# unlikeghost/DeepLearning-MPI

Hardware: AMD Instinct MI355X
Metric: images/sec (whole node) ResNet-50 DDP bs=256/GPU (higher is better)
Workload: dtype bf16; 1 GPU; model=resnet50, global_batch=256, image=224, in_channels=3, per_gpu_batch=256, parallelism=dp1, backend=single, device=cuda, optimizer=SGD(momentum=0.9, wd=1e-5), hipgraph=False

## Files before the change

deeplearning_mpi_amd/csrc/binding/conv_bwd.cpp:

```cpp
#include <c10/hip/HIPCachingAllocator.h>

#include <algorithm>
#include <vector>

#include "common.h"
#include "ops.h"

namespace dlmpi_ext {

using dlmpi::ConvArgs;
using dlmpi::ConvPhase;
using dlmpi::DgradStreamArgs;
using dlmpi::make_fastdiv;
using dlmpi::WgradArgs;

c10::optional<at::Tensor> conv2d_dgrad_pro(const at::Tensor& dy, int N, int P, int Q, int K, int lddy, int dyoff,
                                       const at::Tensor& wT, int C, int R, int S, int stride, int pad, int H, int W,
                                       at::Tensor dx, int lddx, int dxoff, const c10::optional<at::Tensor>& res,
                                       int ldres, int resoff, const c10::optional<at::Tensor>& mask, int ldmask,
                                       int maskoff, const c10::optional<at::Tensor>& z, int ldz, int zoff,
                                       const c10::optional<at::Tensor>& z2, int ldz2, int z2off,
                                       const c10::optional<at::Tensor>& mscale,
                                       const c10::optional<at::Tensor>& mshift,
                                       const c10::optional<at::Tensor>& mbits, bool colsum, int pro,
                                       const c10::optional<at::Tensor>& pk0, const c10::optional<at::Tensor>& pk1,
                                       const c10::optional<at::Tensor>& pz, int ldpz, int pzoff,
                                       const c10::optional<at::Tensor>& bias) {
  require_gpu(dy, "dy");
  if (stride > 2) throw std::runtime_error("conv2d_dgrad: stride <= 2 supported");
  if (bias.has_value() && bias->defined() && (bias->scalar_type() != at::kFloat || bias->numel() < C))
    throw std::runtime_error("conv2d_dgrad: bias must be fp32 [C]");
  ConvArgs a{};
  a.f32 = act_f32(dy, "conv2d_dgrad");
  same_type(dy, wT, "conv2d_dgrad wT");
  same_type(dy, dx, "conv2d_dgrad dx");
  same_type(dy, res, "conv2d_dgrad res");
  same_type(dy, mask, "conv2d_dgrad mask");
  same_type(dy, z, "conv2d_dgrad z");
  same_type(dy, z2, "conv2d_dgrad z2");
  a.x = ptr<uint16_t>(dy);
  a.H = P; a.W = Q; a.C = K; a.ldx = lddy; a.xoff = dyoff;
  a.w = ptr<uint16_t>(wT);
  a.ldw = R * S * K;
  a.S = S;
  a.OH = H; a.OW = W;
  a.so = stride; a.sa = 1;
  a.Nimg = N; a.Kout = C;
  fill_epilogue(a, dx, lddx, dxoff, bias, res, ldres, resoff, c10::nullopt, c10::nullopt, false, c10::nullopt);
  a.vec_store = ((lddx % 8) == 0 && (dxoff % 8) == 0) ? 1 : 0;
  a.mask = optr<uint16_t>(mask);
  a.ldmask = ldmask; a.maskoff = maskoff;
  a.z = optr<uint16_t>(z);
  a.ldz = ldz; a.zoff = zoff;
  a.z2 = optr<uint16_t>(z2);
  a.ldz2 = ldz2; a.z2off = z2off;
  a.mscale = optr<float>(mscale);
  a.mshift = optr<float>(mshift);
  a.mbits = optr<uint8_t>(mbits);
  if (a.mbits && (mbits->numel() != (int64_t)N * H * W * (C / 8) || C % 8))
    throw std::runtime_error("conv2d_dgrad: mask bits must be [N*H*W][C/8]");
  a.nstat = a.z2 ? 3 : 2;
  if (a.z && !a.mask && !a.mscale && !a.mbits)
    throw std::runtime_error("conv2d_dgrad: fused BN statistics need the ReLU mask");
  if (a.mscale && (!a.z || !a.mshift)) throw std::runtime_error("conv2d_dgrad: mask from z needs z, scale, shift");
// ... 32 lines not shown
        (a.z != nullptr) == (mode != 0) && a.vec_store && a.kvalid == C && (lddy | dyoff) % 8 == 0 &&
        (!a.res || (ldres | resoff) % 8 == 0) && fits(M, lddy) && fits(M, lddx) && (!a.res || fits(M, ldres)) &&
        (!a.z || fits(M, ldz)) && (!a.z2 || fits(M, ldz2)) && dx.scalar_type() == at::kBFloat16 &&
        dlmpi_dgrad_stream_plan(M, K, C, mode, a.z2 ? 1 : 0, a.res ? 1 : 0, &sbm, &sbn, &G)) {
      DgradStreamArgs sa{};
      sa.x = ptr<uint16_t>(dy);
      sa.ldx = lddy; sa.xoff = dyoff;
      sa.w = ptr<uint16_t>(wT);
      sa.y = reinterpret_cast<uint16_t*>(a.y);
      sa.ldy = lddx; sa.yoff = dxoff;
      sa.y_bytes = (int)std::min<int64_t>(INT32_MAX, (int64_t)dx.numel() * 2);
      sa.M = (int)M; sa.K = K; sa.Kout = C;
      sa.bias = a.bias;
      sa.res = static_cast<const uint16_t*>(a.res);
      sa.ldres = ldres; sa.resoff = resoff;
      sa.z = static_cast<const uint16_t*>(a.z);
      sa.ldz = ldz; sa.zoff = zoff;
      sa.z2 = static_cast<const uint16_t*>(a.z2);
      sa.ldz2 = ldz2; sa.z2off = z2off;
      sa.mbits = a.mbits;
      sa.mscale = a.mscale; sa.mshift = a.mshift;
      sa.G = G; sa.ntiles = C / sbn; sa.mtiles = (int)ceil_div(M, sbm);
      c10::optional<at::Tensor> st;
      if (a.z) {
        st = at::empty({(int64_t)G, (int64_t)a.nstat, (int64_t)C}, dy.options().dtype(at::kFloat));
        sa.stats = ptr<float>(*st);
      }
      check(dlmpi_conv1x1_dgrad_stream(&sa, sbm, sbn, mode, cur_stream()), "conv2d_dgrad (stream 1x1)");
      g_ran.dgrad_stream = 1;
      return st;
    }
  }
  set_kstep(a, K);
  set_prologue(a, pro, pk0, pk1, pz, ldpz, pzoff);
  TileQuery q{(int64_t)N * H * W / (stride * stride), C, (int64_t)R * S * K / (stride * stride), K, R, S, stride, pad,
              H, W, a.f32, pro};
  q.halo_ok = P == H && Q == W;
  q.pipe_ok = g_sw.pipe_dgrad != 0;
  const Tiles t = select_tiles(q);
  int bm = t.bm, bn = t.bn;
  const int pipe = t.pipe;
  const bool halo = t.halo;
  a.ntiles = ceil_div(C, bn);
  a.nphase = stride * stride;
  int tiles = 0;
  for (int ph = 0; ph < stride; ++ph) {
    for (int pw = 0; pw < stride; ++pw) {
      ConvPhase& p = a.ph[ph * stride + pw];
      const int r0 = (ph + pad) % stride, s0 = (pw + pad) % stride;
      p.P = (H - ph + stride - 1) / stride;
      p.Q = (W - pw + stride - 1) / stride;
      p.Tr = r0 < R ? (R - r0 + stride - 1) / stride : 0;
      p.Ts = s0 < S ? (S - s0 + stride - 1) / stride : 0;
// ... 29 lines not shown
  check(dlmpi_conv_igemm_ex(&a, bm, bn, pipe, cur_stream()), "conv2d_dgrad");
  return stats;
}

c10::optional<at::Tensor> conv2d_dgrad(const at::Tensor& dy, int N, int P, int Q, int K, int lddy, int dyoff,
                                       const at::Tensor& wT, int C, int R, int S, int stride, int pad, int H, int W,
                                       at::Tensor dx, int lddx, int dxoff, const c10::optional<at::Tensor>& res,
                                       int ldres, int resoff, const c10::optional<at::Tensor>& mask, int ldmask,
                                       int maskoff, const c10::optional<at::Tensor>& z, int ldz, int zoff,
                                       const c10::optional<at::Tensor>& z2, int ldz2, int z2off,
                                       const c10::optional<at::Tensor>& mscale,
                                       const c10::optional<at::Tensor>& mshift,
                                       const c10::optional<at::Tensor>& mbits, bool colsum) {
  return conv2d_dgrad_pro(dy, N, P, Q, K, lddy, dyoff, wT, C, R, S, stride, pad, H, W, dx, lddx, dxoff, res, ldres,
                          resoff, mask, ldmask, maskoff, z, ldz, zoff, z2, ldz2, z2off, mscale, mshift, mbits, colsum,
                          0, c10::nullopt, c10::nullopt, c10::nullopt, 0, 0, c10::nullopt);
}

struct PendingReduce {
  at::Tensor ws;
  hipStream_t s;
  dlmpi::WgradReduceEntry e;
};
static std::vector<PendingReduce> g_pending;
static bool g_wgrad_defer = false;
static int g_wgrad_batch = dlmpi::kWgradBatch;
static bool g_defer_direct = true;
static bool g_wgrad_bypass = false;
static int64_t g_reduce_launches = 0;

void wgrad_flush() {
// ... 200 lines not shown
```

deeplearning_mpi_amd/csrc/binding/conv_fwd.cpp:

```cpp
#include <algorithm>
#include <cstdio>
#include <map>
#include <vector>

#include "common.h"

namespace dlmpi_ext {

using dlmpi::ConvArgs;
using dlmpi::ConvPhase;
using dlmpi::FinArgs;
using dlmpi::Stream1x1Args;
using dlmpi::make_fastdiv;

void apply_halo(ConvArgs& a, int N, int bm) {
  ConvPhase& p = a.ph[0];
  int th = 8, tw = 16, tiles_h = 1, tiles_w = 1;
  halo_geom(p.P, p.Q, bm, th, tw, tiles_h, tiles_w);
  a.halo = 1;
  a.th = th;
  a.tw = tw;
  a.tiles_h = tiles_h;
  a.tiles_w = tiles_w;
  a.fd_tw = make_fastdiv((uint32_t)tw);
  a.fd_tilesw = make_fastdiv((uint32_t)tiles_w);
  a.fd_thw = make_fastdiv((uint32_t)(tiles_h * tiles_w));
  p.mtiles = N * tiles_h * tiles_w;
  p.tile_base = 0;
}

static std::map<std::string, TuneCand> g_conv_plans;

static std::string conv_key(const ConvArgs& a, int pass) {
  std::string k = std::to_string(pass);
  auto add = [&](int64_t v) { k += ',' + std::to_string(v); };
  add(a.f32); add(a.Nimg); add(a.H); add(a.W); add(a.C); add(a.ldx); add(a.Kout); add(a.ldw); add(a.S);
  add(a.OH); add(a.OW); add(a.ldy); add(a.so); add(a.sa); add(a.nphase); add(a.kvalid); add(a.vec_store);
  add(a.out_f32); add(a.bias != nullptr); add(a.res != nullptr); add(a.scale != nullptr); add(a.relu);
  add(a.stats != nullptr); add(a.nstat); add(a.mask != nullptr); add(a.mscale != nullptr); add(a.mbits != nullptr);
  add(a.z != nullptr); add(a.z2 != nullptr); add(a.pro);
  for (int i = 0; i < a.nphase; ++i) {
    const ConvPhase& p = a.ph[i];
    add(p.P); add(p.Q); add(p.Tr); add(p.Ts); add(p.dh0); add(p.dw0); add(p.wr0); add(p.ws0);
  }
  return k;
}

static int apply_tiles(ConvArgs& a, int bm, int bn) {
  a.ntiles = ceil_div(a.Kout, bn);
  int t = 0;
  for (int i = 0; i < a.nphase; ++i) {
    ConvPhase& p = a.ph[i];
    p.mtiles = ceil_div((int64_t)a.Nimg * p.P * p.Q, bm);
    p.tile_base = t;
    t += p.mtiles;
// ... 557 lines not shown
```

deeplearning_mpi_amd/csrc/kernels/conv1x1_dgrad_stream.hip:

```cpp
#include "common.h"

namespace dlmpi {

typedef __attribute__((address_space(3))) void dgs_lds_void;

constexpr int dgs_vmcnt(int n) { return (n & 15) | 0x70 | 0xF00 | ((n >> 4) << 14); }
__device__ __forceinline__ void dgs_barrier() { asm volatile("s_waitcnt lgkmcnt(0)\n\ts_barrier" ::: "memory"); }
__device__ __forceinline__ void dgs_glds(const void* g, char* lds) {
  __builtin_amdgcn_global_load_lds(g, (dgs_lds_void*)lds, 16, 0, 0);
}

template <int BN>
__device__ __forceinline__ int dgs_sw(int r) { return BN == 128 ? (r & 15) : ((r >> 1) & 7); }
template <int BN>
__device__ __forceinline__ int dgs_eoff(int r, int col) {
  return r * (2 * BN) + ((((col >> 3) ^ dgs_sw<BN>(r))) << 4) + ((col & 4) << 1);
}

template <int BM, int BN, int KS, int NW, int WGM, int MASK, bool Z2, bool ADB>
__global__ __launch_bounds__(64 * NW) void conv1x1_dgrad_stream_kernel(const DgradStreamArgs a) {
  constexpr bool Z = MASK != 0;
  static_assert(!Z2 || Z, "z2 needs the fused statistics");
  static_assert(BN == 64 || BN == 128, "tile width");
  constexpr bool RES = !(BN == 64 && BM == 64);
// ... 52 lines not shown
  auto issue_a = [&](int mt, char* Ab) {
#pragma unroll
    for (int ks = 0; ks < KS; ++ks)
#pragma unroll
      for (int i = 0; i < AL; ++i) {
        const int m = min(mt * BM + lrow + RP * i, a.M - 1);
        dgs_glds(a.x + (uint32_t)(m * a.ldx + a.xoff + ks * 64 + 8 * jc), Ab + ks * BM * 128 + (RP * i + 8 * wid) * 128);
      }
  };
  auto issue_e = [&](int mt, char* Rb, char* Zb, char* Mb) {
#pragma unroll
    for (int i = 0; i < EL; ++i) {
      const int r = erow + EP * i;
      const int m = min(mt * BM + r, a.M - 1);
      const int gj = ej ^ dgs_sw<BN>(r);
      if (has_res)
        dgs_glds(a.res + (uint32_t)(m * a.ldres + a.resoff + n0 + gj * 8), Rb + i * EP * ERB + wid * 1024);
      if constexpr (Z)
        dgs_glds(a.z + (uint32_t)(m * a.ldz + a.zoff + n0 + gj * 8), Zb + i * EP * ERB + wid * 1024);
      if constexpr (Z2)
        dgs_glds(a.z2 + (uint32_t)(m * a.ldz2 + a.z2off + n0 + gj * 8), Zb + (EZ2_OFF - EZ_OFF) + i * EP * ERB + wid * 1024);
    }
    if constexpr (MASK == 1) {
      if (wid < MB_INSTR) {
        const int piece = wid * 64 + lane;
        const int r = piece * MB_PIECE / MBR;
        const int m = min(mt * BM + r, a.M - 1);
        const uint8_t* src = a.mbits + (uint32_t)(m * (a.Kout >> 3) + (n0 >> 3) + (piece * MB_PIECE) % MBR);
        if constexpr (MB_PIECE == 16) __builtin_amdgcn_global_load_lds(src, (dgs_lds_void*)(Mb + wid * 1024), 16, 0, 0);
        else __builtin_amdgcn_global_load_lds(src, (dgs_lds_void*)(Mb + wid * 256), 4, 0, 0);
      }
    }
// ... 165 lines not shown
    const char* e = getenv("DLMPI_DGS_BLOCKS");
    return e ? atoi(e) : 256;
  }();
  return g_dgs_blocks > 0 ? g_dgs_blocks : env;
}

extern "C" int dlmpi_dgrad_stream_plan(int64_t M, int K, int Kout, int mask_mode, int z2, int has_res, int* bm, int* bn,
                                       int* G) {
  const int blocks = dlmpi_dgs_blocks();
  const int on = g_dgs_override != 0;
  if (!on || M <= 0 || mask_mode < 0 || mask_mode > 2 || (z2 && mask_mode == 0)) return 0;
  if (K == 128 && Kout % 128 == 0) { *bm = 64; *bn = 128; }
  else if (K == 256 && Kout % 128 == 0) {
    *bm = z2 ? 32 : 48;
    *bn = 128;
  }
  else if (K == 512 && Kout % 64 == 0) {
    *bn = 64;
    *bm = (has_res || z2 || mask_mode == 1) ? 32 : 64;
    if (g_dgs_override != 2 && *bm == 32) return 0;
  }
  else return 0;
  const int ntiles = Kout / *bn;
  const int64_t mtiles = (M + *bm - 1) / *bm;
  int target = blocks / ntiles;
  if (target < 8) target = 8;
  *G = (int)(mtiles < target ? mtiles : target);
  return 1;
}

// ... 10 lines not shown
    else hipLaunchKernelGGL((conv1x1_dgrad_stream_kernel<BM_, BN_, KS_, NW_, WGM_, 0, false, ADB_>), grid, blk, 0, s, *a); \
  } while (0)
  if (bm == 64 && bn == 128 && a->K == 128) LAUNCH_DGS(64, 128, 2, 8, 2, false);
  else if (bm == 48 && bn == 128 && a->K == 256 && !a->z2) {
    if (mask_mode == 1) hipLaunchKernelGGL((conv1x1_dgrad_stream_kernel<48, 128, 4, 6, 3, 1, false, false>), grid, dim3(384), 0, s, *a);
    else if (mask_mode == 2) hipLaunchKernelGGL((conv1x1_dgrad_stream_kernel<48, 128, 4, 6, 3, 2, false, false>), grid, dim3(384), 0, s, *a);
    else hipLaunchKernelGGL((conv1x1_dgrad_stream_kernel<48, 128, 4, 6, 3, 0, false, false>), grid, dim3(384), 0, s, *a);
  } else if (bm == 32 && bn == 128 && a->K == 256) {
    if (a->z2) {
      if (mask_mode == 1) hipLaunchKernelGGL((conv1x1_dgrad_stream_kernel<32, 128, 4, 4, 2, 1, true, false>), grid, dim3(256), 0, s, *a);
      else hipLaunchKernelGGL((conv1x1_dgrad_stream_kernel<32, 128, 4, 4, 2, 2, true, false>), grid, dim3(256), 0, s, *a);
    } else if (mask_mode == 1) hipLaunchKernelGGL((conv1x1_dgrad_stream_kernel<32, 128, 4, 4, 2, 1, false, false>), grid, dim3(256), 0, s, *a);
    else if (mask_mode == 2) hipLaunchKernelGGL((conv1x1_dgrad_stream_kernel<32, 128, 4, 4, 2, 2, false, false>), grid, dim3(256), 0, s, *a);
    else hipLaunchKernelGGL((conv1x1_dgrad_stream_kernel<32, 128, 4, 4, 2, 0, false, false>), grid, dim3(256), 0, s, *a);
  }
  else if (bm == 32 && bn == 64 && a->K == 512) LAUNCH_DGS(32, 64, 8, 4, 2, false);
  else if (bm == 64 && bn == 64 && a->K == 512 && !a->z2 && !a->res) {
    if (mask_mode == 2) hipLaunchKernelGGL((conv1x1_dgrad_stream_kernel<64, 64, 8, 8, 2, 2, false, false>), grid, dim3(512), 0, s, *a);
    else if (mask_mode == 0) hipLaunchKernelGGL((conv1x1_dgrad_stream_kernel<64, 64, 8, 8, 2, 0, false, false>), grid, dim3(512), 0, s, *a);
    else return hipErrorInvalidValue;
  }
  else return hipErrorInvalidValue;
#undef LAUNCH_DGS
  return hipGetLastError();
}
```

deeplearning_mpi_amd/csrc/kernels/conv_igemm.hip:

```cpp
#include <cstdlib>
#include <type_traits>

#include "common.h"

namespace dlmpi {

typedef __attribute__((address_space(3))) void lds_void;

__device__ __forceinline__ void glds16(const void* g, char* lds_wave_base) {
  __builtin_amdgcn_global_load_lds(g, (lds_void*)lds_wave_base, 16, 0, 0);
}

template <int BM, int BN, int NT, int WM>
struct EpiSmem {
  static constexpr int NP0 = BM < 128 ? 1 : (BM / 64 < WM / 16 ? BM / 64 : WM / 16);
  static constexpr int NP = (WM / 16) % NP0 == 0 ? NP0 : WM / 16;
  static constexpr int CS_LD = BN + 4;
  static constexpr int EPI = (BM / NP) * CS_LD * 4;
  static constexpr int RED = (NT / (BN / 8)) * 3 * BN * 4;
  static constexpr int bytes = EPI > RED ? EPI : RED;
};

template <int NT, int NF>
__device__ __forceinline__ bool splitk_combine(const ConvArgs& a, f32x4* acc, char* smem, int tid, int mt, int nt) {
// ... 16 lines not shown
    __builtin_amdgcn_fence(__ATOMIC_ACQUIRE, "agent");
    asm volatile("s_waitcnt vmcnt(0)" ::: "memory");
    __hip_atomic_store(a.sk_tk + tile, 0, __ATOMIC_RELAXED, __HIP_MEMORY_SCOPE_AGENT);
  }
  __syncthreads();
  const f32x4* base = reinterpret_cast<const f32x4*>(a.sk_slab) + tile * S * NF * NT + tid;
#pragma unroll
  for (int i = 0; i < NF; ++i) acc[i] = f32x4{0.f, 0.f, 0.f, 0.f};
  for (int sp = 0; sp < S; ++sp)
#pragma unroll
    for (int i = 0; i < NF; ++i) acc[i] += base[((int64_t)sp * NF + i) * NT];
  __syncthreads();
  return true;
}

template <int BM, int BN, int NT, int WGM, int WGN, typename T, bool HALO>
__device__ __forceinline__ void conv_epilogue(const ConvArgs& a, const ConvPhase& ph,
                                              f32x4 (&acc)[BM / WGM / 16][BN / WGN / 16], char* smem, int tid,
                                              int m0, int n0, int mt, int hn, int hh0, int hw0) {
  constexpr int WM = BM / WGM, WN = BN / WGN;
  constexpr int TM = WM / 16, TN = WN / 16;
  constexpr int NP = EpiSmem<BM, BN, NT, WM>::NP;
  constexpr int CS_LD = EpiSmem<BM, BN, NT, WM>::CS_LD;
  static_assert(WM % (16 * NP) == 0 || NP == 1, "epilogue pass must split every wave's rows evenly");
  const int lane = tid & 63;
  const int wid = __builtin_amdgcn_readfirstlane(tid >> 6);
  const int wm = wid / WGN, wn = wid % WGN;
  const int fr = lane & 15, fg = lane >> 4;
  const int PQ = ph.P * ph.Q;
  const int M = a.Nimg * PQ;
  float* Cs = reinterpret_cast<float*>(smem);
// ... 21 lines not shown
  if (h) __syncthreads();
#pragma unroll
  for (int mi = 0; mi < HT; ++mi)
#pragma unroll
    for (int ni = 0; ni < TN; ++ni)
#pragma unroll
      for (int r = 0; r < 4; ++r)
        Cs[(wm * HM + mi * 16 + fg * 4 + r) * CS_LD + wn * WN + ni * 16 + fr] = acc[h * HT + mi][ni][r];
  __syncthreads();
  constexpr int EPI_UNROLL = BM >= 256 ? 1 : 2;
#pragma unroll EPI_UNROLL
  for (int rr = rg; rr < BM / NP; rr += RG) {
    const int r = (rr / HM) * WM + h * HM + (rr % HM);
    const int m = m0 + r;
    int64_t pix;
    if constexpr (HALO) {
      const int pr = (int)fdiv((uint32_t)r, a.fd_tw), pc = r - pr * a.tw;
      const int oh = hh0 + pr, ow = hw0 + pc;
      if (r >= a.th * a.tw || oh >= ph.P || ow >= ph.Q || !cvalid) continue;
      pix = ((int64_t)hn * a.OH + oh * a.so + ph.oh0) * a.OW + ow * a.so + ph.ow0;
    } else {
      if (m >= M || !cvalid) continue;
    }
    float v[8];
    const f32x4 v0 = *reinterpret_cast<const f32x4*>(Cs + rr * CS_LD + cg * 8);
    const f32x4 v1 = *reinterpret_cast<const f32x4*>(Cs + rr * CS_LD + cg * 8 + 4);
#pragma unroll
    for (int e = 0; e < 4; ++e) { v[e] = v0[e] + bias[e]; v[e + 4] = v1[e] + bias[e + 4]; }
    if (a.stats && !bwd) {
#pragma unroll
      for (int e = 0; e < 8; ++e) {
        const float rv = stored<T>(v[e]);
        s1[e] += rv;
        s2[e] += rv * rv;
      }
    }
    if (a.scale) {
#pragma unroll
      for (int e = 0; e < 8; ++e) v[e] = v[e] * a.scale[c0 + e] + a.shift[c0 + e];
    }
    if constexpr (!HALO) {
      const uint32_t n_img = fdiv((uint32_t)m, ph.fdPQ);
      const uint32_t rem = (uint32_t)m - n_img * PQ;
      const uint32_t p = fdiv(rem, ph.fdQ);
      const uint32_t q = rem - p * ph.Q;
      pix = ((int64_t)n_img * a.OH + (int)p * a.so + ph.oh0) * a.OW + (int)q * a.so + ph.ow0;
    }
    if (a.res) {
      float rr8[8];
      load8(static_cast<const T*>(a.res) + pix * a.ldres + a.resoff + c0, rr8);
#pragma unroll
      for (int e = 0; e < 8; ++e) v[e] += rr8[e];
    }
    if (a.relu) {
#pragma unroll
      for (int e = 0; e < 8; ++e) v[e] = fmaxf(v[e], 0.f);
    }
    if (bwd) {
      float zz[8];
      if (a.z) load8(static_cast<const T*>(a.z) + pix * a.ldz + a.zoff + c0, zz);
      if (a.mbits) {
        const uint32_t b = a.mbits[pix * (a.Kout >> 3) + (c0 >> 3)];
#pragma unroll
        for (int e = 0; e < 8; ++e) v[e] = (b >> e) & 1u ? v[e] : 0.f;
      } else if (a.mask) {
// ... 602 lines not shown
        for (int q = 0; q < MH; ++q)
#pragma unroll
          for (int ni = 0; ni < TN; ++ni)
            if (h * MH + q < TM)
              acc[h * MH + q][ni] = __builtin_amdgcn_mfma_f32_16x16x32_bf16(af[q], bfr[ni], acc[h * MH + q][ni], 0, 0, 0);
      }
    }
  };
  for (int ks = 0; ks < nk; ks += STAGES) {
    step(ks, std::integral_constant<int, 0>{});
    if (ks + 1 < nk) step(ks + 1, std::integral_constant<int, 1>{});
    if constexpr (STAGES == 3)
      if (ks + 2 < nk) step(ks + 2, std::integral_constant<int, 2>{});
  }
  __syncthreads();
  conv_epilogue<BM, BN, NT, WGM, WGN, uint16_t, false>(a, ph, acc, smem, tid, m0, n0, mt, 0, 0, 0);
}

template <int BM, int BN, int WGM>
__global__ __launch_bounds__(256) __attribute__((amdgpu_waves_per_eu(2, 2))) void conv_halo_pipe_kernel(const ConvArgs a) {
  constexpr int NW = 4, NT = 256, WGN = NW / WGM;
  constexpr int WM = BM / WGM, WN = BN / WGN, TM = WM / 16, TN = WN / 16;
  constexpr int RP = NT / 8;
  constexpr int BL = BN / RP;
  constexpr int HALO_ROWS = BM == 256 ? 352 : 192;
  constexpr int HL = HALO_ROWS / RP;
  constexpr int A_BYTES = HALO_ROWS * 128, B_BYTES = BN * 128;
  constexpr int SB = A_BYTES + 2 * B_BYTES;
  constexpr int EPI_NEED = EpiSmem<BM, BN, NT, WM>::bytes;
  constexpr int SMEM = SB > EPI_NEED ? SB : EPI_NEED;
  static_assert(HALO_ROWS % RP == 0 && BN % RP == 0 && TM >= 1 && TN >= 1, "tile shape");
// ... 299 lines not shown
      }
#pragma unroll
      for (int ni = 0; ni < TN; ++ni) {
        const int r = wn * WN + ni * 16 + fr;
        bfr[ni] = *reinterpret_cast<const bf16x8*>(Bs + r * 128 + ((ch ^ (r & 7)) << 4));
      }
#pragma unroll
      for (int mi = 0; mi < TM; ++mi)
#pragma unroll
        for (int ni = 0; ni < TN; ++ni)
          acc[mi][ni] = __builtin_amdgcn_mfma_f32_16x16x32_bf16(af[mi], bfr[ni], acc[mi][ni], 0, 0, 0);
    }
    if (k + 1 < nk) commit(k + 1, (k + 1) & 1);
    __syncthreads();
  }
  conv_epilogue<BM, BN, NT, WGM, WGN, uint16_t, false>(a, ph, acc, smem, tid, m0, 0, (int)mt, 0, 0, 0);
}

}

using namespace dlmpi;

template <int BM, int BN>
static hipError_t launch_tile(const ConvArgs* a, dim3 grid, hipStream_t s) {
  if (a->pro == 3) {
    if constexpr (BM == 128 && BN == 64) hipLaunchKernelGGL((conv_igemm_kernel<BM, BN, false, 2, 3>), grid, dim3(256), 0, s, *a);
    else return hipErrorInvalidValue;
  } else if (a->C < 64) hipLaunchKernelGGL((conv_igemm_kernel<BM, BN, true, 2>), grid, dim3(256), 0, s, *a);
  else hipLaunchKernelGGL((conv_igemm_kernel<BM, BN, false, 2>), grid, dim3(256), 0, s, *a);
  return hipSuccess;
}
// ... 122 lines not shown
```

deeplearning_mpi_amd/csrc/kernels/dlmpi_kernels.h:

```cpp
#pragma once
#include <hip/hip_runtime_api.h>
#include <stdint.h>

namespace dlmpi {

struct FastDiv {
  uint32_t d, mul, shr;
};
inline FastDiv make_fastdiv(uint32_t d) {
  FastDiv f;
  f.d = d;
  uint32_t l = 0;
  while ((1ull << l) < d) ++l;
  f.mul = (uint32_t)((((1ull << 32) * ((1ull << l) - d)) / d) + 1);
  f.shr = l;
  return f;
}

struct FinArgs {
  int mode;
  double count;
  const float* gamma;
  const float* beta;
  float* running_mean;
// ... 27 lines not shown
  int up2;
  int Cup;
};

struct DgradStreamArgs {
  const uint16_t* x;
  int ldx, xoff;
  const uint16_t* w;
  uint16_t* y;
  int ldy, yoff;
  int y_bytes;
  int M, K, Kout;
  const float* bias;
  const uint16_t* res;
  int ldres, resoff;
  const uint16_t* z;
  int ldz, zoff;
  const uint16_t* z2;
  int ldz2, z2off;
  const uint8_t* mbits;
  const float* mscale;
  const float* mshift;
  float* stats;
  int G, ntiles, mtiles;
};

struct ConvPhase {
  int P, Q;
  int Tr, Ts;
  int dh0, dhs, dw0, dws;
// ... 324 lines not shown
```

deeplearning_mpi_amd/models/engine.py:

```python
from __future__ import annotations

import contextlib
import os
from typing import NamedTuple, Optional

import torch
import torch.nn as nn

from ..ops.act import Act, Deferred, padc
from ..ops.backend import make_backend
from ..utils.arena import ParamArena
from ..utils.profiler import range as trace_range


@contextlib.contextmanager
def grad_side(be, *tensors):
    side = getattr(be, "side_stream", None)
    if side is None:
        yield
        return
    cur = torch.cuda.current_stream()
    side.wait_stream(cur)
    torch.cuda.set_stream(side)
    try:
# ... 23 lines not shown
            record_on(stream, o.buf)
        elif isinstance(o, (tuple, list)):
            record_on(stream, *o)


_STREAM_HOLD = True

_OUTER_DGRAD = True
_HEAD_DGRAD = True

DEFER_BN_WGRAD = True

DUAL_DGRAD = True
DUAL_MIN_ROWS = 2 * 256 * 28 * 28
DUAL_WGRAD_PRO = True

FUSE_APPLY = True
FUSE_APPLY_MAX_K = 256
FUSE_APPLY_3X3 = True

WGRAD_TAIL_MAIN = True


def img_rows(a, n0: int, n1: int):
    if a is None:
        return None
    if isinstance(a, Deferred):
        return Deferred(a.kind, img_rows(a.src, n0, n1), img_rows(a.z, n0, n1), a.k0, a.k1)
    hw = a.H * a.W
    return Act(a.buf[n0 * hw:n1 * hw], n1 - n0, a.H, a.W, a.C, a.off)
# ... 76 lines not shown
            self.h_fwd = arena.add_compute(w, (self.Kp, R, S, self.Cp), (K, R, S, C), (0, 2, 3, 1))
            self.h_dg = arena.add_compute(w, (self.Cp, R, S, self.Kp), (C, R, S, K), (1, 2, 3, 0)) \
                if need_dgrad else None
        self.bias = conv.bias
        self._bias_pad = None

    dual = False

    def dy_slot(self, ctx) -> Optional[Act]:
        if not self.dual or ctx is None:
            return None
        z = ctx[1]
        if z is None or z.off != z.C or z.ld != 2 * z.C:
            return None
        return Act(z.buf, z.N, z.H, z.W, z.C, 0)

    def out_hw(self, H, W):
        return ((H + 2 * self.pad - self.R) // self.stride + 1, (W + 2 * self.pad - self.S) // self.stride + 1)

    def _weight_fwd(self):
        return self.arena.get_compute(self.h_fwd)

    def prep_input(self, be, x: torch.Tensor) -> Act:
        return be.nchw_to_nhwc(x, self.Cp)

    def _wgrad(self, be, dz: Act, x: Act):
        be.conv_wgrad(dz, x, self.R, self.S, self.stride, self.pad, self.arena.grad_flat(self.conv.weight),
                      self.Cin, self.K)

    def _bias_vec(self):
# ... 108 lines not shown
        shift = (bn.bias.data if bn.affine else 0.0) - bn.running_mean * scale
        if self.bias is not None:
            shift = shift + self.bias.data * scale
        be.conv_fwd(x, wf, self.Kp, self.R, self.S, self.stride, self.pad, y, res=res, scale=scale.contiguous(),
                    shift=shift.contiguous(), relu=self.relu)
        return y, None

    @staticmethod
    def fuse_spec(ctx, z2=None) -> BwdFuse:
        x, z, y, mean, invstd, scale, shift, has_res, mbits = ctx
        if has_res or z2 is not None:
            return BwdFuse(None if mbits is not None else y, z, z2, mbits=mbits)
        return BwdFuse(None, z, None, scale, shift)

    def bwd(self, be, ctx, dy: Act, need_dx=True, dx_res: Act = None, dyr_out: Act = None, ymask: Act = None,
            use_own_mask=True, pre=None, k2=1, fuse_next=None, colsum=False, before_res=None, dx_out: Act = None):
        ar = self.arena
        bn = self.bn
        dg_in, dg_w, dg_b = None, None, None
        if bn is not None and need_dx and pre is not None and dyr_out is None and self.dual:
            x, z = ctx[0], ctx[1]
            if (z.off == z.C and z.ld == 2 * z.C and dy.off == 0 and dy.ld == z.ld
                    and dy.buf.data_ptr() == z.buf.data_ptr()):
                mean, invstd = ctx[3], ctx[4]
                gam = bn.weight.data if bn.affine else None
                dzd = be.bn_bwd_deferred(dy, z, mean, invstd, gam, ar.grad_flat(bn.weight) if bn.affine else None,
                                         ar.grad_flat(bn.bias) if bn.affine else None, pre=pre, k2=k2)
                with grad_side(be, *bufs(dzd, x)):
                    if bn.affine:
                        ar.ready(bn.weight, bn.bias)
                    if self.bias is not None:
# ... 46 lines not shown
                        be.channel_sum(dz, ar.grad_flat(self.bias))
                    else:
                        tmp = torch.empty(self.Kp, dtype=be.dt, device=dz.device)
                        be.fill_(tmp, 0.0)
                        be.channel_sum(dz, tmp)
                        if getattr(self, "_kidx", None) is None or self._kidx.device != dz.device:
                            self._kidx = torch.arange(self.K, device=dz.device)
                        be.gather_(ar.grad_flat(self.bias), tmp, self._kidx, accumulate=True)
                    ar.ready(self.bias)
                self._wgrad(be, dz, x)
                ar.ready(self.conv.weight)
        if not need_dx:
            return None
        if before_res is not None:
            before_res()
        if dx_out is not None:
            assert (dx_out.N, dx_out.H, dx_out.W, dx_out.C) == (x.N, x.H, x.W, self.Cp), (dx_out, x, self.Cp)
            dx = dx_out
        else:
            dx = Act.empty(x.N, x.H, x.W, self.Cp, be.act_dtype, x.device)
        if dg_in is not None:
            part = be.conv_dgrad(dg_in, dg_w, self.Cp, 1, 1, 1, 0, dx, res=dx_res, fuse=fuse_next, colsum=colsum,
                                 bias=dg_b)
            return (dx, part) if (fuse_next is not None or colsum) else dx
        if (self.K == 1 and self.R == 1 and self.S == 1 and self.stride == 1 and dx_res is None and not colsum
                and fuse_next is not None and fuse_next.scale is not None and fuse_next.z2 is None
                and hasattr(be, "outer_dgrad_bn") and _OUTER_DGRAD):
            part = be.outer_dgrad_bn(be.materialize(dz), ar.get_compute(self.h_dg), self.Kp, dx, fuse_next)
            return dx, part
        if (2 <= self.K <= 4 and self.R == 1 and self.S == 1 and self.stride == 1 and dx_res is None and not colsum
                and fuse_next is not None and fuse_next.scale is not None and fuse_next.z2 is None
                and hasattr(be, "head_dgrad_bn") and _HEAD_DGRAD):
            part = be.head_dgrad_bn(be.materialize(dz), self.K, ar.get_compute(self.h_dg), self.Kp, dx, fuse_next)
            return dx, part
        part = be.conv_dgrad(dz, ar.get_compute(self.h_dg), self.Cp, self.R, self.S, self.stride, self.pad, dx,
                             res=dx_res, fuse=fuse_next, colsum=colsum)
        return (dx, part) if (fuse_next is not None or colsum) else dx


class S2DConvUnit(ConvUnit):

    CS = 4

    def __init__(self, arena: ParamArena, conv, bn=None, relu=True):
        w = conv.weight
        K, Cin, R, S = w.shape
        assert conv.stride == (2, 2) and conv.padding[0] == conv.padding[1] and conv.groups == 1
        assert Cin <= self.CS and conv.dilation == (1, 1)
        self.arena, self.conv, self.bn, self.relu = arena, conv, bn, relu
        self.linear = False
        self.K, self.Cin, self.R0, self.S0, self.pad0 = K, Cin, R, S, conv.padding[0]
# ... 230 lines not shown
```

deeplearning_mpi_amd/models/resnet.py:

```python
from __future__ import annotations


import torch
import torch.nn as nn
import torch.nn.functional as F

from ..ops.act import Act, padc
from .engine import PendingApply, BwdFuse, ConvUnit, EngineModule, S2DConvUnit, record_on, resolve


def conv3x3(i, o, stride=1):
    return nn.Conv2d(i, o, 3, stride, 1, bias=False)


def conv1x1(i, o, stride=1):
    return nn.Conv2d(i, o, 1, stride, 0, bias=False)


class BasicBlock(nn.Module):
    expansion = 1

    def __init__(self, inplanes, planes, stride=1, downsample=None):
        super().__init__()
        self.conv1 = conv3x3(inplanes, planes, stride)
# ... 103 lines not shown
        return y, (ctxs, cd)

    def fuse_spec(self, st):
        ctxs, cd = st
        return ConvUnit.fuse_spec(ctxs[-1], z2=cd[1] if cd is not None else None)

    def out_slot(self, st):
        return self.u[-1].dy_slot(st[0][-1])

    def bwd(self, be, st, dy: Act, pre=None, fuse_prev=None, fuse_inner=False, dx_out=None):
        ctxs, cd = st
        slot = lambda k: self.u[k].dy_slot(ctxs[k])
        ylast = ctxs[-1][2]
        n = len(self.u)
        spec = lambda k: ConvUnit.fuse_spec(ctxs[k])
        if pre is not None:
            br = getattr(be, "branch_stream", None) if self.ud is not None else None
            if br is not None:
                main = torch.cuda.current_stream()
                br.wait_stream(main)
                with torch.cuda.stream(br):
                    dres = self.ud.bwd(be, cd, dy, pre=pre, k2=2)
                record_on(br, dy, pre)
            dh, part = self.u[-1].bwd(be, ctxs[-1], dy, pre=pre, k2=1, fuse_next=spec(n - 2), dx_out=slot(n - 2))
            for k in range(n - 2, 0, -1):
                dh, part = self.u[k].bwd(be, ctxs[k], dh, pre=part, fuse_next=spec(k - 1), dx_out=slot(k - 1))
            join = None
            if br is not None:
                def join():
                    main.wait_stream(br)
                    record_on(main, dres)
                if not _LATE_JOIN:
                    join()
                    join = None
            elif self.ud is not None:
                dres = self.ud.bwd(be, cd, dy, pre=pre, k2=2)
            else:
                dres = dy
            return self.u[0].bwd(be, ctxs[0], dh, dx_res=dres, pre=part, fuse_next=fuse_prev, before_res=join,
                                 dx_out=dx_out)
        inner = fuse_inner or any(c[2] is None for c in ctxs[:-1])
        if self.ud is None:
            dyr = Act.empty(dy.N, dy.H, dy.W, dy.C, be.act_dtype, dy.device)
            dh = self.u[-1].bwd(be, ctxs[-1], dy, dyr_out=dyr, fuse_next=spec(n - 2) if inner else None,
                                dx_out=slot(n - 2))
        else:
            dyr = None
            dh = self.u[-1].bwd(be, ctxs[-1], dy, fuse_next=spec(n - 2) if inner else None, dx_out=slot(n - 2))
        part = None
        if inner:
            dh, part = dh
        for k in range(n - 2, 0, -1):
            if inner:
                dh, part = self.u[k].bwd(be, ctxs[k], dh, pre=part, fuse_next=spec(k - 1), dx_out=slot(k - 1))
            else:
                dh = self.u[k].bwd(be, ctxs[k], dh, dx_out=slot(k - 1))
        if self.ud is not None:
            dres = self.ud.bwd(be, cd, dy, ymask=ylast)
        else:
            dres = dyr
        out = self.u[0].bwd(be, ctxs[0], dh, dx_res=dres, pre=part, fuse_next=fuse_prev, dx_out=dx_out)
        return out


class ResNet(EngineModule):
    def __init__(self, block, layers, num_classes=1000, in_channels=3):
        super().__init__()
        self.inplanes = 64
        self.in_channels = in_channels
        self.conv1 = nn.Conv2d(in_channels, 64, kernel_size=7, stride=2, padding=3, bias=False)
        self.bn1 = nn.BatchNorm2d(64)
        self.relu = nn.ReLU(inplace=True)
        self.maxpool = nn.MaxPool2d(kernel_size=3, stride=2, padding=1)
        self.layer1 = self._make_layer(block, 64, layers[0])
        self.layer2 = self._make_layer(block, 128, layers[1], stride=2)
        self.layer3 = self._make_layer(block, 256, layers[2], stride=2)
# ... 128 lines not shown
```

deeplearning_mpi_amd/ops/backend.py:

```python
from __future__ import annotations

import os
import weakref
import struct

import torch
import torch.nn.functional as F

from .act import Act, Deferred


_AUX_STREAMS = {}
_BACKENDS = weakref.WeakSet()


def _new_aux_stream(idx, C, role):
    with torch.cuda.device(idx):
        st = torch.cuda.ExternalStream(C.create_stream(), device=torch.device("cuda", idx))
        C.set_aux_stream(st.cuda_stream, role)
    return st


def _aux_stream(device, C, role):
    idx = device.index if device.index is not None else torch.cuda.current_device()
# ... 144 lines not shown
        x, y = xp.z, xp.y
        r = self.C.conv3x3_fwd_bn_apply(x.buf, x.N, x.H, x.W, x.ld, x.off, w, z.buf, z.ld, z.off, bias, stats,
                                        xp.scale, xp.shift, y.buf, y.ld, y.off, float(count), gamma, beta, rm, rv,
                                        float(momentum), float(eps), scale, shift, save_mean, save_invstd)
        if r < 0:
            self.bn_apply(xp.z, xp.scale, xp.shift, None, True, y)
            self.conv_fwd_bn(y, w, K, 3, 3, 1, 1, z, bias, stats, count, gamma, beta, rm, rv, momentum, eps, scale,
                             shift, save_mean, save_invstd)

    def conv_fwd_bnbwd(self, x: Act, w, K, R, S, stride, pad, y: Act, fuse):
        z = fuse.z
        return self.C.conv2d_fwd_bnbwd(x.buf, x.N, x.H, x.W, x.C, x.ld, x.off, w, K, R, S, stride, pad, y.buf, y.ld,
                                       y.off, z.buf, z.ld, z.off, fuse.scale, fuse.shift)

    def conv_dgrad(self, dy: Act, wT, C, R, S, stride, pad, dx: Act, res: Act = None, fuse=None, colsum=False,
                   bias=None):
        m, z, z2, sc, sh, mb = fuse if fuse is not None else (None, None, None, None, None, None)

        def t(a):
            return (a.buf, a.ld, a.off) if a is not None else (None, 0, 0)

        dy = self.materialize(dy)
        return self.C.conv2d_dgrad_pro(dy.buf, dy.N, dy.H, dy.W, dy.C, dy.ld, dy.off, wT, C, R, S, stride, pad, dx.H,
                                       dx.W, dx.buf, dx.ld, dx.off, *t(res), *t(m), *t(z), *t(z2), sc, sh, mb,
                                       bool(colsum and fuse is None), 0, None, None, None, 0, 0, bias)

    def dual_weights(self, wT, C, K, coef):
        w2 = torch.empty(C, 2 * K, dtype=self.act_dtype, device=self.device)
        b = torch.empty(C, dtype=torch.float32, device=self.device)
        self.C.dual_dgrad_weights(wT, C, K, coef, w2, b)
        return w2, b

    def convT_fwd(self, x: Act, wf, Cout, y: Act, bias=None):
        self.C.convT2x2_fwd(x.buf, x.N, x.H, x.W, x.C, x.ld, x.off, wf, Cout, y.buf, y.ld, y.off, bias)

    def wgrad_defer(self, on: bool):
        self.C.set_wgrad_defer(bool(on))

    def wgrad_flush(self):
        self.C.wgrad_flush()
# ... 343 lines not shown
            out = F.relu(out)
        self._store(y, out)

    def conv_fwd_bn(self, x, w, K, R, S, stride, pad, z: Act, bias, stats, count, gamma, beta, rm, rv, momentum,
                    eps, scale, shift, save_mean, save_invstd):
        self.conv_fwd(x, w, K, R, S, stride, pad, z, bias=bias, stats=stats)
        self.bn_finalize(stats, stats.shape[0], K, count, gamma, beta, rm, rv, momentum, eps, scale, shift,
                         save_mean, save_invstd)

    def dual_weights(self, wT, C, K, coef):
        w = wT.reshape(C, K).to(self.dt)
        c = coef.to(self.dt)
        w2 = torch.cat([w * c[0], w * c[1]], 1).to(self.act_dtype)
        return w2, (w * c[2]).sum(1)

    def conv_dgrad(self, dy, wT, C, R, S, stride, pad, dx: Act, res=None, fuse=None, colsum=False, bias=None):
        dy = self.materialize(dy)
        K = dy.C
        wk = wT.view(C, R, S, K).permute(3, 0, 1, 2).to(self.dt)
        g = torch.nn.grad.conv2d_input((dx.N, C, dx.H, dx.W), wk, dy.nchw().to(self.dt), stride, pad)
        if bias is not None:
            g = g + bias.to(self.dt).view(1, -1, 1, 1)
        if res is not None:
            g = g + res.nchw().to(self.dt)
        if fuse is None:
            self._store(dx, g)
            if colsum:
                v = dx.nhwc().to(self.dt)
                return torch.stack([v.sum((0, 1, 2)), (v * v).sum((0, 1, 2))]).unsqueeze(0)
            return None
        m, z, z2, sc, sh, mb = fuse
        if mb is not None:
            g = g * self._unpack_bits(mb, z).permute(0, 3, 1, 2)
        elif m is not None:
            g = g * (m.nchw() > 0)
        else:
            keep = (z.nhwc().to(self.dt) * sc + sh) > 0
            g = g * keep.permute(0, 3, 1, 2)
# ... 485 lines not shown
```

Baseline: 13690 images/sec.

## Compute strided-1x1 downsample dgrad compactly and fuse upsampled residual into main dgrad

For the stride-2 1x1 downsample branch, the input gradient is now computed at the output resolution as a plain 1x1 stride-1 dgrad, giving a compact tensor, instead of a full-resolution dx that is mostly zeros. The main branch's dgrad epilogue then adds this compact residual by mapping each output pixel to the subsampled row and reading a zero page for odd positions, signalled by a negative ldres or a res_sub field. A new 64x64 tile configuration is added to the streamed 1x1 dgrad kernel for K=256, and the reference backend is updated to match. The aim is to cut the FLOPs and memory traffic of the downsample dgrad and its residual read. In exchange it adds index arithmetic in the epilogues and disables the halo and pipelined tile paths when the compact residual is used.

```diff
diff --git a/deeplearning_mpi_amd/csrc/binding/conv_bwd.cpp b/deeplearning_mpi_amd/csrc/binding/conv_bwd.cpp
--- a/deeplearning_mpi_amd/csrc/binding/conv_bwd.cpp
+++ b/deeplearning_mpi_amd/csrc/binding/conv_bwd.cpp
@@ -25,8 +25,9 @@
                                        const c10::optional<at::Tensor>& mbits, bool colsum, int pro,
                                        const c10::optional<at::Tensor>& pk0, const c10::optional<at::Tensor>& pk1,
                                        const c10::optional<at::Tensor>& pz, int ldpz, int pzoff,
-                                       const c10::optional<at::Tensor>& bias) {
+                                       const c10::optional<at::Tensor>& bias, int res_sub) {
   require_gpu(dy, "dy");
+  if (res_sub != 1 && res_sub != 2) throw std::runtime_error("conv2d_dgrad: res_sub must be 1 or 2");
   if (stride > 2) throw std::runtime_error("conv2d_dgrad: stride <= 2 supported");
   if (bias.has_value() && bias->defined() && (bias->scalar_type() != at::kFloat || bias->numel() < C))
     throw std::runtime_error("conv2d_dgrad: bias must be fp32 [C]");
@@ -48,6 +49,13 @@
   a.Nimg = N; a.Kout = C;
   fill_epilogue(a, dx, lddx, dxoff, bias, res, ldres, resoff, c10::nullopt, c10::nullopt, false, c10::nullopt);
   a.vec_store = ((lddx % 8) == 0 && (dxoff % 8) == 0) ? 1 : 0;
+  const int res_P = (H + 1) / 2, res_Q = (W + 1) / 2;
+  if (res_sub == 2) {
+    if (!a.res) throw std::runtime_error("conv2d_dgrad: res_sub without a residual");
+    const int64_t rrows = (int64_t)N * res_P * res_Q;
+    if (ldres < resoff + C || resoff < 0 || res->numel() < (rrows - 1) * ldres + resoff + C)
+      throw std::runtime_error("conv2d_dgrad: compact residual must be [N*ceil(H/2)*ceil(W/2)][ldres]");
+  }
   a.mask = optr<uint16_t>(mask);
   a.ldmask = ldmask; a.maskoff = maskoff;
   a.z = optr<uint16_t>(z);
@@ -110,6 +118,9 @@
       sa.bias = a.bias;
       sa.res = static_cast<const uint16_t*>(a.res);
       sa.ldres = ldres; sa.resoff = resoff;
+      sa.res_sub = res_sub; sa.res_P = res_P; sa.res_Q = res_Q;
+      sa.fdHW = make_fastdiv((uint32_t)(H * W));
+      sa.fdW = make_fastdiv((uint32_t)W);
       sa.z = static_cast<const uint16_t*>(a.z);
       sa.ldz = ldz; sa.zoff = zoff;
       sa.z2 = static_cast<const uint16_t*>(a.z2);
@@ -129,10 +140,11 @@
   }
   set_kstep(a, K);
   set_prologue(a, pro, pk0, pk1, pz, ldpz, pzoff);
+  if (res_sub == 2) a.ldres = -ldres;
   TileQuery q{(int64_t)N * H * W / (stride * stride), C, (int64_t)R * S * K / (stride * stride), K, R, S, stride, pad,
               H, W, a.f32, pro};
-  q.halo_ok = P == H && Q == W;
-  q.pipe_ok = g_sw.pipe_dgrad != 0;
+  q.halo_ok = P == H && Q == W && res_sub != 2;
+  q.pipe_ok = g_sw.pipe_dgrad != 0 && res_sub != 2;
   const Tiles t = select_tiles(q);
   int bm = t.bm, bn = t.bn;
   const int pipe = t.pipe;
@@ -192,7 +204,7 @@
                                        const c10::optional<at::Tensor>& mbits, bool colsum) {
   return conv2d_dgrad_pro(dy, N, P, Q, K, lddy, dyoff, wT, C, R, S, stride, pad, H, W, dx, lddx, dxoff, res, ldres,
                           resoff, mask, ldmask, maskoff, z, ldz, zoff, z2, ldz2, z2off, mscale, mshift, mbits, colsum,
-                          0, c10::nullopt, c10::nullopt, c10::nullopt, 0, 0, c10::nullopt);
+                          0, c10::nullopt, c10::nullopt, c10::nullopt, 0, 0, c10::nullopt, 1);
 }
 
 struct PendingReduce {
diff --git a/deeplearning_mpi_amd/csrc/binding/conv_fwd.cpp b/deeplearning_mpi_amd/csrc/binding/conv_fwd.cpp
--- a/deeplearning_mpi_amd/csrc/binding/conv_fwd.cpp
+++ b/deeplearning_mpi_amd/csrc/binding/conv_fwd.cpp
@@ -38,7 +38,7 @@
   add(a.OH); add(a.OW); add(a.ldy); add(a.so); add(a.sa); add(a.nphase); add(a.kvalid); add(a.vec_store);
   add(a.out_f32); add(a.bias != nullptr); add(a.res != nullptr); add(a.scale != nullptr); add(a.relu);
   add(a.stats != nullptr); add(a.nstat); add(a.mask != nullptr); add(a.mscale != nullptr); add(a.mbits != nullptr);
-  add(a.z != nullptr); add(a.z2 != nullptr); add(a.pro);
+  add(a.z != nullptr); add(a.z2 != nullptr); add(a.pro); add(a.ldres < 0);
   for (int i = 0; i < a.nphase; ++i) {
     const ConvPhase& p = a.ph[i];
     add(p.P); add(p.Q); add(p.Tr); add(p.Ts); add(p.dh0); add(p.dw0); add(p.wr0); add(p.ws0);
diff --git a/deeplearning_mpi_amd/csrc/kernels/conv1x1_dgrad_stream.hip b/deeplearning_mpi_amd/csrc/kernels/conv1x1_dgrad_stream.hip
--- a/deeplearning_mpi_amd/csrc/kernels/conv1x1_dgrad_stream.hip
+++ b/deeplearning_mpi_amd/csrc/kernels/conv1x1_dgrad_stream.hip
@@ -90,8 +90,19 @@
       const int r = erow + EP * i;
       const int m = min(mt * BM + r, a.M - 1);
       const int gj = ej ^ dgs_sw<BN>(r);
-      if (has_res)
-        dgs_glds(a.res + (uint32_t)(m * a.ldres + a.resoff + n0 + gj * 8), Rb + i * EP * ERB + wid * 1024);
+      if (has_res) {
+        const uint16_t* rsrc;
+        if (a.res_sub == 2) {
+          const uint32_t n = fdiv((uint32_t)m, a.fdHW), rem = (uint32_t)m - n * a.fdHW.d;
+          const uint32_t h = fdiv(rem, a.fdW), w = rem - h * a.fdW.d;
+          const uint32_t rrow = (n * a.res_P + (h >> 1)) * a.res_Q + (w >> 1);
+          rsrc = ((h | w) & 1u) ? reinterpret_cast<const uint16_t*>(zp)
+                                : a.res + (uint32_t)(rrow * a.ldres + a.resoff + n0 + gj * 8);
+        } else {
+          rsrc = a.res + (uint32_t)(m * a.ldres + a.resoff + n0 + gj * 8);
+        }
+        dgs_glds(rsrc, Rb + i * EP * ERB + wid * 1024);
+      }
       if constexpr (Z)
         dgs_glds(a.z + (uint32_t)(m * a.ldz + a.zoff + n0 + gj * 8), Zb + i * EP * ERB + wid * 1024);
       if constexpr (Z2)
@@ -287,6 +298,11 @@
   else if (K == 256 && Kout % 128 == 0) {
     *bm = z2 ? 32 : 48;
     *bn = 128;
+  }
+  else if (K == 256 && Kout % 64 == 0) {
+    if (has_res || z2 || mask_mode == 1) return 0;
+    *bm = 64;
+    *bn = 64;
   }
   else if (K == 512 && Kout % 64 == 0) {
     *bn = 64;
@@ -327,6 +343,16 @@
     else if (mask_mode == 2) hipLaunchKernelGGL((conv1x1_dgrad_stream_kernel<32, 128, 4, 4, 2, 2, false, false>), grid, dim3(256), 0, s, *a);
     else hipLaunchKernelGGL((conv1x1_dgrad_stream_kernel<32, 128, 4, 4, 2, 0, false, false>), grid, dim3(256), 0, s, *a);
   }
+  else if (bm == 64 && bn == 64 && a->K == 256 && !a->z2 && !a->res) {
+    const bool adb = g_dgs_override == 3;
+    if (mask_mode == 2) {
+      if (adb) hipLaunchKernelGGL((conv1x1_dgrad_stream_kernel<64, 64, 4, 8, 2, 2, false, true>), grid, dim3(512), 0, s, *a);
+      else hipLaunchKernelGGL((conv1x1_dgrad_stream_kernel<64, 64, 4, 8, 2, 2, false, false>), grid, dim3(512), 0, s, *a);
+    } else if (mask_mode == 0) {
+      if (adb) hipLaunchKernelGGL((conv1x1_dgrad_stream_kernel<64, 64, 4, 8, 2, 0, false, true>), grid, dim3(512), 0, s, *a);
+      else hipLaunchKernelGGL((conv1x1_dgrad_stream_kernel<64, 64, 4, 8, 2, 0, false, false>), grid, dim3(512), 0, s, *a);
+    } else return hipErrorInvalidValue;
+  }
   else if (bm == 32 && bn == 64 && a->K == 512) LAUNCH_DGS(32, 64, 8, 4, 2, false);
   else if (bm == 64 && bn == 64 && a->K == 512 && !a->z2 && !a->res) {
     if (mask_mode == 2) hipLaunchKernelGGL((conv1x1_dgrad_stream_kernel<64, 64, 8, 8, 2, 2, false, false>), grid, dim3(512), 0, s, *a);
diff --git a/deeplearning_mpi_amd/csrc/kernels/conv_igemm.hip b/deeplearning_mpi_amd/csrc/kernels/conv_igemm.hip
--- a/deeplearning_mpi_amd/csrc/kernels/conv_igemm.hip
+++ b/deeplearning_mpi_amd/csrc/kernels/conv_igemm.hip
@@ -54,7 +54,7 @@
   return true;
 }
 
-template <int BM, int BN, int NT, int WGM, int WGN, typename T, bool HALO>
+template <int BM, int BN, int NT, int WGM, int WGN, typename T, bool HALO, bool RSUB = !HALO>
 __device__ __forceinline__ void conv_epilogue(const ConvArgs& a, const ConvPhase& ph,
                                               f32x4 (&acc)[BM / WGM / 16][BN / WGN / 16], char* smem, int tid,
                                               int m0, int n0, int mt, int hn, int hh0, int hw0) {
@@ -106,11 +106,13 @@
     const int r = (rr / HM) * WM + h * HM + (rr % HM);
     const int m = m0 + r;
     int64_t pix;
+    int on, oy, ox;
     if constexpr (HALO) {
       const int pr = (int)fdiv((uint32_t)r, a.fd_tw), pc = r - pr * a.tw;
       const int oh = hh0 + pr, ow = hw0 + pc;
       if (r >= a.th * a.tw || oh >= ph.P || ow >= ph.Q || !cvalid) continue;
-      pix = ((int64_t)hn * a.OH + oh * a.so + ph.oh0) * a.OW + ow * a.so + ph.ow0;
+      on = hn; oy = oh * a.so + ph.oh0; ox = ow * a.so + ph.ow0;
+      pix = ((int64_t)on * a.OH + oy) * a.OW + ox;
     } else {
       if (m >= M || !cvalid) continue;
     }
@@ -136,11 +138,25 @@
       const uint32_t rem = (uint32_t)m - n_img * PQ;
       const uint32_t p = fdiv(rem, ph.fdQ);
       const uint32_t q = rem - p * ph.Q;
-      pix = ((int64_t)n_img * a.OH + (int)p * a.so + ph.oh0) * a.OW + (int)q * a.so + ph.ow0;
+      on = (int)n_img; oy = (int)p * a.so + ph.oh0; ox = (int)q * a.so + ph.ow0;
+      pix = ((int64_t)on * a.OH + oy) * a.OW + ox;
     }
     if (a.res) {
       float rr8[8];
-      load8(static_cast<const T*>(a.res) + pix * a.ldres + a.resoff + c0, rr8);
+      int64_t rpix = pix;
+      int ldr = a.ldres;
+      bool rzero = false;
+      if constexpr (RSUB) {
+        int p2 = a.OH + 1, q2 = a.OW + 1;
+        asm volatile("" : "+v"(p2), "+v"(q2), "+v"(ldr));
+        const bool sub = ldr < 0;
+        ldr = sub ? -ldr : ldr;
+        rpix = sub ? ((int64_t)on * (p2 >> 1) + (oy >> 1)) * (q2 >> 1) + (ox >> 1) : pix;
+        rzero = sub && ((oy | ox) & 1);
+      }
+      const T* rp = static_cast<const T*>(a.res) + rpix * ldr + a.resoff + c0;
+      if (rzero) rp = reinterpret_cast<const T*>(g_zero_page);
+      load8(rp, rr8);
 #pragma unroll
       for (int e = 0; e < 8; ++e) v[e] += rr8[e];
     }
@@ -773,7 +789,7 @@
       if (ks + 2 < nk) step(ks + 2, std::integral_constant<int, 2>{});
   }
   __syncthreads();
-  conv_epilogue<BM, BN, NT, WGM, WGN, uint16_t, false>(a, ph, acc, smem, tid, m0, n0, mt, 0, 0, 0);
+  conv_epilogue<BM, BN, NT, WGM, WGN, uint16_t, false, false>(a, ph, acc, smem, tid, m0, n0, mt, 0, 0, 0);
 }
 
 template <int BM, int BN, int WGM>
@@ -1103,7 +1119,7 @@
     if (k + 1 < nk) commit(k + 1, (k + 1) & 1);
     __syncthreads();
   }
-  conv_epilogue<BM, BN, NT, WGM, WGN, uint16_t, false>(a, ph, acc, smem, tid, m0, 0, (int)mt, 0, 0, 0);
+  conv_epilogue<BM, BN, NT, WGM, WGN, uint16_t, false, false>(a, ph, acc, smem, tid, m0, 0, (int)mt, 0, 0, 0);
 }
 
 }
diff --git a/deeplearning_mpi_amd/csrc/kernels/dlmpi_kernels.h b/deeplearning_mpi_amd/csrc/kernels/dlmpi_kernels.h
--- a/deeplearning_mpi_amd/csrc/kernels/dlmpi_kernels.h
+++ b/deeplearning_mpi_amd/csrc/kernels/dlmpi_kernels.h
@@ -65,6 +65,8 @@
   const float* bias;
   const uint16_t* res;
   int ldres, resoff;
+  int res_sub, res_P, res_Q;
+  FastDiv fdHW, fdW;
   const uint16_t* z;
   int ldz, zoff;
   const uint16_t* z2;
diff --git a/deeplearning_mpi_amd/models/engine.py b/deeplearning_mpi_amd/models/engine.py
--- a/deeplearning_mpi_amd/models/engine.py
+++ b/deeplearning_mpi_amd/models/engine.py
@@ -61,6 +61,8 @@
 DUAL_DGRAD = True
 DUAL_MIN_ROWS = 2 * 256 * 28 * 28
 DUAL_WGRAD_PRO = True
+
+COMPACT_DS = True
 
 FUSE_APPLY = True
 FUSE_APPLY_MAX_K = 256
@@ -167,6 +169,10 @@
         if z is None or z.off != z.C or z.ld != 2 * z.C:
             return None
         return Act(z.buf, z.N, z.H, z.W, z.C, 0)
+
+    def compact_dx(self) -> bool:
+        return (COMPACT_DS and not self.linear and self.R == 1 and self.S == 1 and self.stride == 2
+                and self.pad == 0 and self.h_dg is not None)
 
     def out_hw(self, H, W):
         return ((H + 2 * self.pad - self.R) // self.stride + 1, (W + 2 * self.pad - self.S) // self.stride + 1)
@@ -305,7 +311,8 @@
         return BwdFuse(None, z, None, scale, shift)
 
     def bwd(self, be, ctx, dy: Act, need_dx=True, dx_res: Act = None, dyr_out: Act = None, ymask: Act = None,
-            use_own_mask=True, pre=None, k2=1, fuse_next=None, colsum=False, before_res=None, dx_out: Act = None):
+            use_own_mask=True, pre=None, k2=1, fuse_next=None, colsum=False, before_res=None, dx_out: Act = None,
+            res_sub=1, compact=False):
         ar = self.arena
         bn = self.bn
         dg_in, dg_w, dg_b = None, None, None
@@ -382,6 +389,12 @@
             return None
         if before_res is not None:
             before_res()
+        if compact:
+            assert self.compact_dx() and dx_res is None and fuse_next is None and not colsum and dx_out is None
+            dz = be.materialize(dz)
+            dx = Act.empty(dz.N, dz.H, dz.W, self.Cp, be.act_dtype, dz.device)
+            be.conv_dgrad(dz, ar.get_compute(self.h_dg), self.Cp, 1, 1, 1, 0, dx)
+            return dx
         if dx_out is not None:
             assert (dx_out.N, dx_out.H, dx_out.W, dx_out.C) == (x.N, x.H, x.W, self.Cp), (dx_out, x, self.Cp)
             dx = dx_out
@@ -389,7 +402,7 @@
             dx = Act.empty(x.N, x.H, x.W, self.Cp, be.act_dtype, x.device)
         if dg_in is not None:
             part = be.conv_dgrad(dg_in, dg_w, self.Cp, 1, 1, 1, 0, dx, res=dx_res, fuse=fuse_next, colsum=colsum,
-                                 bias=dg_b)
+                                 bias=dg_b, res_sub=res_sub)
             return (dx, part) if (fuse_next is not None or colsum) else dx
         if (self.K == 1 and self.R == 1 and self.S == 1 and self.stride == 1 and dx_res is None and not colsum
                 and fuse_next is not None and fuse_next.scale is not None and fuse_next.z2 is None
@@ -402,7 +415,7 @@
             part = be.head_dgrad_bn(be.materialize(dz), self.K, ar.get_compute(self.h_dg), self.Kp, dx, fuse_next)
             return dx, part
         part = be.conv_dgrad(dz, ar.get_compute(self.h_dg), self.Cp, self.R, self.S, self.stride, self.pad, dx,
-                             res=dx_res, fuse=fuse_next, colsum=colsum)
+                             res=dx_res, fuse=fuse_next, colsum=colsum, res_sub=res_sub)
         return (dx, part) if (fuse_next is not None or colsum) else dx
 
 
diff --git a/deeplearning_mpi_amd/models/resnet.py b/deeplearning_mpi_amd/models/resnet.py
--- a/deeplearning_mpi_amd/models/resnet.py
+++ b/deeplearning_mpi_amd/models/resnet.py
@@ -141,13 +141,15 @@
         ylast = ctxs[-1][2]
         n = len(self.u)
         spec = lambda k: ConvUnit.fuse_spec(ctxs[k])
+        compact = self.ud is not None and self.ud.compact_dx()
+        sub = 2 if compact else 1
         if pre is not None:
             br = getattr(be, "branch_stream", None) if self.ud is not None else None
             if br is not None:
                 main = torch.cuda.current_stream()
                 br.wait_stream(main)
                 with torch.cuda.stream(br):
-                    dres = self.ud.bwd(be, cd, dy, pre=pre, k2=2)
+                    dres = self.ud.bwd(be, cd, dy, pre=pre, k2=2, compact=compact)
                 record_on(br, dy, pre)
             dh, part = self.u[-1].bwd(be, ctxs[-1], dy, pre=pre, k2=1, fuse_next=spec(n - 2), dx_out=slot(n - 2))
             for k in range(n - 2, 0, -1):
@@ -161,11 +163,11 @@
                     join()
                     join = None
             elif self.ud is not None:
-                dres = self.ud.bwd(be, cd, dy, pre=pre, k2=2)
+                dres = self.ud.bwd(be, cd, dy, pre=pre, k2=2, compact=compact)
             else:
                 dres = dy
             return self.u[0].bwd(be, ctxs[0], dh, dx_res=dres, pre=part, fuse_next=fuse_prev, before_res=join,
-                                 dx_out=dx_out)
+                                 dx_out=dx_out, res_sub=sub)
         inner = fuse_inner or any(c[2] is None for c in ctxs[:-1])
         if self.ud is None:
             dyr = Act.empty(dy.N, dy.H, dy.W, dy.C, be.act_dtype, dy.device)
@@ -183,10 +185,10 @@
             else:
                 dh = self.u[k].bwd(be, ctxs[k], dh, dx_out=slot(k - 1))
         if self.ud is not None:
-            dres = self.ud.bwd(be, cd, dy, ymask=ylast)
+            dres = self.ud.bwd(be, cd, dy, ymask=ylast, compact=compact)
         else:
             dres = dyr
-        out = self.u[0].bwd(be, ctxs[0], dh, dx_res=dres, pre=part, fuse_next=fuse_prev, dx_out=dx_out)
+        out = self.u[0].bwd(be, ctxs[0], dh, dx_res=dres, pre=part, fuse_next=fuse_prev, dx_out=dx_out, res_sub=sub)
         return out
 
 
diff --git a/deeplearning_mpi_amd/ops/backend.py b/deeplearning_mpi_amd/ops/backend.py
--- a/deeplearning_mpi_amd/ops/backend.py
+++ b/deeplearning_mpi_amd/ops/backend.py
@@ -182,7 +182,9 @@
                                        y.off, z.buf, z.ld, z.off, fuse.scale, fuse.shift)
 
     def conv_dgrad(self, dy: Act, wT, C, R, S, stride, pad, dx: Act, res: Act = None, fuse=None, colsum=False,
-                   bias=None):
+                   bias=None, res_sub=1):
+        if res_sub == 2:
+            assert res is not None and (res.N, res.H, res.W) == (dx.N, (dx.H + 1) // 2, (dx.W + 1) // 2), (res, dx)
         m, z, z2, sc, sh, mb = fuse if fuse is not None else (None, None, None, None, None, None)
 
         def t(a):
@@ -191,7 +193,7 @@
         dy = self.materialize(dy)
         return self.C.conv2d_dgrad_pro(dy.buf, dy.N, dy.H, dy.W, dy.C, dy.ld, dy.off, wT, C, R, S, stride, pad, dx.H,
                                        dx.W, dx.buf, dx.ld, dx.off, *t(res), *t(m), *t(z), *t(z2), sc, sh, mb,
-                                       bool(colsum and fuse is None), 0, None, None, None, 0, 0, bias)
+                                       bool(colsum and fuse is None), 0, None, None, None, 0, 0, bias, int(res_sub))
 
     def dual_weights(self, wT, C, K, coef):
         w2 = torch.empty(C, 2 * K, dtype=self.act_dtype, device=self.device)
@@ -565,14 +567,25 @@
         w2 = torch.cat([w * c[0], w * c[1]], 1).to(self.act_dtype)
         return w2, (w * c[2]).sum(1)
 
-    def conv_dgrad(self, dy, wT, C, R, S, stride, pad, dx: Act, res=None, fuse=None, colsum=False, bias=None):
+    def conv_dgrad(self, dy, wT, C, R, S, stride, pad, dx: Act, res=None, fuse=None, colsum=False, bias=None,
+                   res_sub=1):
         dy = self.materialize(dy)
         K = dy.C
         wk = wT.view(C, R, S, K).permute(3, 0, 1, 2).to(self.dt)
-        g = torch.nn.grad.conv2d_input((dx.N, C, dx.H, dx.W), wk, dy.nchw().to(self.dt), stride, pad)
+        if R == 1 and S == 1 and pad == 0 and stride == 2:
+            gc = torch.nn.grad.conv2d_input((dx.N, C, dy.H, dy.W), wk, dy.nchw().to(self.dt), 1, 0)
+            g = torch.zeros(dx.N, C, dx.H, dx.W, dtype=gc.dtype, device=gc.device)
+            g[:, :, ::2, ::2] = gc
+        else:
+            g = torch.nn.grad.conv2d_input((dx.N, C, dx.H, dx.W), wk, dy.nchw().to(self.dt), stride, pad)
         if bias is not None:
             g = g + bias.to(self.dt).view(1, -1, 1, 1)
-        if res is not None:
+        if res is not None and res_sub == 2:
+            assert (res.N, res.H, res.W) == (dx.N, (dx.H + 1) // 2, (dx.W + 1) // 2), (res, dx)
+            up = torch.zeros_like(g)
+            up[:, :, ::2, ::2] = res.nchw().to(self.dt)
+            g = g + up
+        elif res is not None:
             g = g + res.nchw().to(self.dt)
         if fuse is None:
             self._store(dx, g)
```

Result: no change. 13770 images/sec (median of 6 runs) (+0.6%).
